# holstegelab/otter

Hardware: AMD Instinct MI355X
Metric: regions/sec (otter assemble) on synthetic TR BED+BAM, 1/2/4/8 MI355X (higher is better)
Workload: dtype i16

## Files before the change

### otter_amd/csrc/otg_chain.hpp

```cpp
#pragma once
#include "otg_common.hpp"
#include <cstddef>
#include <cstdlib>

struct OtgCounters {
  struct Tier { uint32_t ticket, overflow; };
  struct ExactEdit {
    uint32_t wf_ticket, tier_ticket[OTG_MYERS_TIERS];
    Tier wide, last;
    struct Routes { uint32_t len[OTG_MYERS_TIERS + 1], wf_len; } routes;
  } exact_edit;
  struct ExactAffine {
    uint32_t seg[OTG_REG_TIERS + 2];
    uint32_t reg_overflow, reg_ticket[OTG_REG_TIERS], bound_ticket;
    Tier a, b, c;
    unsigned long long visited, unused_, reg_timing[7];
  } exact_affine;
  struct AdaptiveEdit { Tier packed1024, packed4096, packed16384, bytes2048, bytes16384, last; } adaptive_edit;
  struct AdaptiveAffine { Tier win256, win1024, win4096, bytes1024, last; } adaptive_affine;
};
static_assert(offsetof(OtgCounters, exact_affine.visited) % 8 == 0 && offsetof(OtgCounters, exact_affine.reg_timing) % 8 == 0, "64-bit atomics need 8-byte alignment");
static_assert(offsetof(OtgCounters, exact_affine.reg_timing) - offsetof(OtgCounters, exact_affine.visited) == 16, "wfa_affine_reg.hip adds its clock sums at visited + 2 .. visited + 8");
static_assert(sizeof(OtgCounters::ExactEdit::Routes) <= 16 * sizeof(uint32_t), "ctx->edit_hist holds 16 words per kind of pass");

template <class G>
G* otg_counters(otg_ctx* ctx, G OtgCounters::*group, size_t bytes = sizeof(G))
{
  const bool fresh = !ctx->pool[SLOT_COUNTERS].p;
  OtgCounters* c = (OtgCounters*)otg_slot(ctx, SLOT_COUNTERS, sizeof(OtgCounters));
  if (!c) return nullptr;
  ctx->last_chain = (int)((const char*)&(c->*group) - (const char*)c);
  const hipError_t e = fresh ? hipMemsetAsync(c, 0, sizeof(OtgCounters), ctx->stream) : hipMemsetAsync(&(c->*group), 0, bytes, ctx->stream);
  if (e != hipSuccess) { otg_fail(ctx, OTG_ERR_HIP, "zeroing the chain counters failed"); return nullptr; }
  return &(c->*group);
}
inline unsigned long long* otg_affine_visited(otg_ctx* ctx) { OtgCounters* c = (OtgCounters*)ctx->pool[SLOT_COUNTERS].p; return c ? &c->exact_affine.visited : nullptr; }

inline int otg_timer_add(otg_ctx* ctx, float* kernel_ms, uint64_t* launches)
{
  if (!kernel_ms) return OTG_OK;
  HIP_TRY(ctx, hipEventSynchronize(ctx->ev1));
  float ms = 0;
  HIP_TRY(ctx, hipEventElapsedTime(&ms, ctx->ev0, ctx->ev1));
  *kernel_ms += ms;
  if (launches) *launches += 1;
  return OTG_OK;
}

struct OtgTodo {
  const uint32_t *list, *n; uint32_t imm;
  void next(const uint32_t* gave_up, const uint32_t* len) { list = gave_up; n = len; imm = 0; }
};

inline int otg_env_int(const char* name, int dflt) { const char* v = getenv(name); return v ? atoi(v) : dflt; }
inline bool otg_env_set(const char* name) { return getenv(name) != nullptr; }
// ... 1 lines not shown
```

### otter_amd/csrc/wfa_affine.hip

```cpp
#include "wfa_affine_common.hpp"
#include "wfa_affine_reg.hpp"
#include "otg_chain.hpp"
#include "otg_match_queue.hpp"
#include <algorithm>
#include <cstdlib>
#include <mutex>
#include <vector>

using namespace otg_affine;

namespace {

template <int WPB>
__global__ __launch_bounds__(WPB * 64) void wfa_affine_kernel(
    const uint8_t* __restrict__ arena, const otg_align_task* __restrict__ tasks,
    const uint32_t* __restrict__ todo, const uint32_t* __restrict__ n_todo_ptr, uint32_t n_todo_imm,
    int xs, int oes, int es, int g,
    int32_t* __restrict__ scores, const uint64_t* __restrict__ cig_off, uint32_t* __restrict__ cig_len,
    uint8_t* __restrict__ cig_arena, uint64_t* __restrict__ cells,
    uint32_t* __restrict__ ticket, uint32_t* __restrict__ n_overflow, uint32_t* __restrict__ overflow_list,
    AffWs ws)
{
  constexpr int QCAP = 2048;
  __shared__ int s_lo[WPB][3][64];
// ... 707 lines not shown
  const uint32_t a = seg[0], n = seg[1] - seg[0];
  for (uint32_t i = blockIdx.x * blockDim.x + threadIdx.x; i < n; i += gridDim.x * blockDim.x) out[i] = sorted[a + i];
  if (blockIdx.x == 0 && threadIdx.x == 0) *n_out = n;
}

}

int otg_launch_affine(otg_ctx* ctx, const uint8_t* d_arena, const otg_align_task* d_tasks, uint32_t n_tasks,
                      int x, int o, int e, int32_t* d_scores, const uint64_t* d_cig_off, uint32_t* d_cig_len,
                      uint8_t* d_cig_arena, uint64_t* d_cells)
{
  return otg_launch_affine_todo(ctx, d_arena, d_tasks, nullptr, nullptr, n_tasks, x, o, e, d_scores, d_cig_off, d_cig_len, d_cig_arena, d_cells);
}

int otg_launch_affine_todo(otg_ctx* ctx, const uint8_t* d_arena, const otg_align_task* d_tasks, const uint32_t* d_todo,
                           const uint32_t* d_n_todo, uint32_t n_tasks, int x, int o, int e, int32_t* d_scores,
                           const uint64_t* d_cig_off, uint32_t* d_cig_len, uint8_t* d_cig_arena, uint64_t* d_cells,
                           float* kernel_ms, uint64_t* launches)
{
  if (n_tasks == 0) return OTG_OK;
  ctx->affine_last = {};
  if (ctx->heur_strategy == OTG_HEURISTIC_WFADAPTIVE)
    return otg_launch_affine_adaptive_todo(ctx, d_arena, d_tasks, d_todo, d_n_todo, n_tasks, x, o, e, d_scores, d_cig_off, d_cig_len, d_cig_arena, d_cells,
                                           kernel_ms, launches);
  int g, xs, oes, es;
  if (int rc = affine_penalties(ctx, x, o, e, &g, &xs, &oes, &es)) return rc;
  OtgCounters::ExactAffine* const cnt = otg_counters(ctx, &OtgCounters::exact_affine, offsetof(OtgCounters::ExactAffine, visited));
  uint32_t* todo = (uint32_t*)otg_slot(ctx, SLOT_TODO, 4 * (size_t)n_tasks * sizeof(uint32_t));
  if (!cnt || !todo) return OTG_ERR_HIP;

  const size_t maxlen = ((size_t)ctx->max_seq_len + 4095) & ~(size_t)4095;
  AffWs ws = aff_ws_common(maxlen, xs, oes, es);
  ws.dbg = otg_env_set("OTG_DEBUG") ? 1 : 0; ws.visited = &cnt->visited;
  aff_ws_layout(ws, true);

  static const bool no_v3 = otg_env_set("OTG_NO_AFFINE_V3");
  static const bool no_bound = otg_env_set("OTG_NO_AFFINE_BOUND");
  static const int reg_mask_env = otg_env_int("OTG_AFFINE_REG", 31);
  static const int shape_env = otg_env_int("OTG_REG_SHAPE", 0);
  const int shape[OTG_REG_TIERS] = {(shape_env / 10000) % 10, (shape_env / 1000) % 10, (shape_env / 100) % 10, (shape_env / 10) % 10, shape_env % 10};
  const bool bounded = !no_v3 && es == 1 && xs == 2 && oes == 4 && !no_bound;
  int reg_mask = !bounded ? 0 : (maxlen <= 4096 ? (reg_mask_env & ~16) : reg_mask_env) & 31;

  constexpr int NWA = 4;
  constexpr int WPB = 4;
  AffWs wsA = ws, wsB = ws, wsC = ws, wr[OTG_REG_TIERS];
  uint32_t wavesA = 0, wavesB = 0, gridC = 2, blocks[OTG_REG_TIERS] = {0, 0, 0, 0, 0};
  const uint32_t ncu = (uint32_t)ctx->n_cu;
  {
    std::lock_guard<std::mutex> alloc_lock(otg_device_mutex(ctx->device));
    size_t free_b = 0, total_b = 0;
    HIP_TRY(ctx, hipMemGetInfo(&free_b, &total_b));
    const size_t budget = std::min<size_t>((size_t)(total_b * 0.2), (size_t)((free_b + ctx->pool[SLOT_WF_WS].cap) * 0.8));
    auto fit = [&](uint32_t& nwaves, size_t& slab) {
      while (nwaves > 1 && (ws.off_slab + slab) * (size_t)nwaves > budget) {
        if (slab > ((size_t)4 << 20)) slab /= 2; else nwaves = (nwaves + 1) / 2;
      }
    };
    auto diamond_slab = [&](size_t window) { return std::min<size_t>((size_t)(0.2 * (double)maxlen * (double)maxlen), window * window * 5 / 8) + (1 << 16); };
    wavesA = ncu * 2; size_t slabA = diamond_slab(4096);
    fit(wavesA, slabA);
    aff_ws_slab(wsA, slabA);
    wavesB = maxlen > 8192 ? ncu : ncu / 2; size_t slabB = diamond_slab(12288);
    fit(wavesB, slabB);
    aff_ws_slab(wsB, slabB);
    size_t slabC = std::min<size_t>((size_t)2 * maxlen * (size_t)(ws.nrows), budget / (gridC * WPB));
// ... 162 lines not shown
      std::vector<uint32_t> ids;
      if (d_todo) {
        if (d_n_todo) HIP_TRY(ctx, hipMemcpy(&n_live, d_n_todo, 4, hipMemcpyDeviceToHost)); else n_live = n_tasks;
        ids.resize(n_live);
        if (n_live) HIP_TRY(ctx, hipMemcpy(ids.data(), d_todo, (size_t)n_live * 4, hipMemcpyDeviceToHost));
      } else { n_live = n_tasks; ids.resize(n_live); for (uint32_t i = 0; i < n_live; ++i) ids[i] = i; }
      double su2 = 0, ss2 = 0; uint64_t hist[6] = {0, 0, 0, 0, 0, 0}, n_ok = 0;
      for (uint32_t q = 0; q < n_live; ++q) {
        const int32_t U = hb[ids[q]], sc = hs[ids[q]];
        if (U < 0 || U >= 0x40000000 || sc <= 0) continue;
        const double u = (double)U * g, r = u / (double)sc;
        su2 += u * u; ss2 += (double)sc * sc; ++n_ok;
        ++hist[r <= 1.0 ? 0 : r <= 1.02 ? 1 : r <= 1.05 ? 2 : r <= 1.1 ? 3 : r <= 1.2 ? 4 : 5];
      }
      if (n_ok) fprintf(stderr, "[otg] affine: bound / final score over %llu alignments: == 1: %.1f %%, <= 1.02: %.1f %%, <= 1.05: %.1f %%, <= 1.1: %.1f %%, <= 1.2: %.1f %%, above: %.1f %%; diamond cells outside the exact score's diamond: %.1f %%\n",
                        (unsigned long long)n_ok, 100.0 * hist[0] / n_ok, 100.0 * hist[1] / n_ok, 100.0 * hist[2] / n_ok, 100.0 * hist[3] / n_ok, 100.0 * hist[4] / n_ok, 100.0 * hist[5] / n_ok,
                        100.0 * (su2 - ss2) / su2);
    }
    if (h.reg_overflow && dbg_bound && bounded && reg_mask) {
      const uint32_t nshow = std::min<uint32_t>(h.reg_overflow, 24u);
      std::vector<uint32_t> ids(nshow);
      HIP_TRY(ctx, hipMemcpy(ids.data(), todo + 3 * (size_t)n_tasks, nshow * sizeof(uint32_t), hipMemcpyDeviceToHost));
      for (uint32_t i = 0; i < nshow; ++i) {
        otg_align_task t; int32_t U = 0, sc = 0;
        HIP_TRY(ctx, hipMemcpy(&t, d_tasks + ids[i], sizeof(t), hipMemcpyDeviceToHost));
        HIP_TRY(ctx, hipMemcpy(&U, dbg_bound + ids[i], sizeof(U), hipMemcpyDeviceToHost));
        HIP_TRY(ctx, hipMemcpy(&sc, d_scores + ids[i], sizeof(sc), hipMemcpyDeviceToHost));
        fprintf(stderr, "[otg] affine:   left its register tier: task %u, pattern %u, text %u, ends-free %d (pattern begin / end %d / %d, text begin / end %d / %d), bound %d, score %d\n",
                ids[i], t.pattern_len, t.text_len, t.endsfree, t.pattern_begin_free, t.pattern_end_free, t.text_begin_free, t.text_end_free, U, sc);
      }
    }
#ifdef OTG_REG_TIMING
    const unsigned long long* tm = h.reg_timing;
    HIP_TRY(ctx, hipMemsetAsync(cnt->reg_timing, 0, sizeof(h.reg_timing), ctx->stream));
    if (tm[5]) fprintf(stderr, "[otg] register tiers, clock ticks per wave and score: preamble %.0f sweep %.0f (%.2f slot visits) drain+fold %.0f exports %.0f barrier %.0f; %llu wave-scores\n",
                       (double)tm[0] / tm[5], (double)tm[1] / tm[5], (double)tm[6] / tm[5], (double)tm[2] / tm[5], (double)tm[3] / tm[5], (double)tm[4] / tm[5], tm[5]);
#endif
  }
  return otg_timer_add(ctx, kernel_ms, launches);
}

extern "C" int otg_affine_last_routing(otg_ctx* ctx, uint32_t n_tasks, int32_t* bound_out, int8_t* routed_out, int8_t* finished_out,
                                       uint32_t* counts_out, uint32_t* lists_out)
{
  const char* const who = "otg_affine_last_routing";
  if (!ctx) return otg_fail(nullptr, OTG_ERR_ARG, "%s: NULL context", who);
  if (!bound_out || !routed_out || !finished_out || !counts_out != !lists_out) return otg_fail(ctx, OTG_ERR_ARG, "%s: NULL argument", who);
  const otg_ctx::AffineLast& L = ctx->affine_last;
  if (ctx->heur_strategy != OTG_HEURISTIC_NONE) return otg_fail(ctx, OTG_ERR_ARG, "%s: the context's heuristic is WFadaptive; only the exact gap-affine chain is accounted for", who);
  if (ctx->last_chain != (int)offsetof(OtgCounters, exact_affine) || !ctx->pool[SLOT_COUNTERS].p || !ctx->pool[SLOT_TODO].p)
    return otg_fail(ctx, OTG_ERR_ARG, "%s: the last tier chain launched on this context was not the exact gap-affine chain", who);
  if (n_tasks == 0 || n_tasks != L.n_tasks) return otg_fail(ctx, OTG_ERR_ARG, "%s: the last gap-affine launch had %u tasks, not %u", who, L.n_tasks, n_tasks);
  if (L.sublist) return otg_fail(ctx, OTG_ERR_ARG, "%s: the last gap-affine launch worked on a list of task slots (the region pipeline's), not on a whole batch", who);
  if (ctx->pool[SLOT_TODO].cap < 4 * (size_t)n_tasks * sizeof(uint32_t) || (L.bounded && ctx->pool[SLOT_BT_POOL].cap < (size_t)n_tasks * sizeof(int32_t)))
    return otg_fail(ctx, OTG_ERR_ARG, "%s: the workspaces of the last gap-affine launch have been released", who);
  if (!L.scores_at || L.scores_at != ctx->pool[SLOT_SCORES].p || ctx->pool[SLOT_SCORES].cap < (size_t)n_tasks * sizeof(int32_t))
    return otg_fail(ctx, OTG_ERR_ARG, "%s: the scores of the last gap-affine launch are not in the context's score buffer (any more)", who);
  HIP_TRY(ctx, hipSetDevice(ctx->device));
  HIP_TRY(ctx, hipStreamSynchronize(ctx->stream));
  OtgCounters::ExactAffine c;
  HIP_TRY(ctx, hipMemcpy(&c, &((const OtgCounters*)ctx->pool[SLOT_COUNTERS].p)->exact_affine, sizeof(c), hipMemcpyDeviceToHost));
  std::vector<uint32_t> lists(4 * (size_t)n_tasks);
  HIP_TRY(ctx, hipMemcpy(lists.data(), ctx->pool[SLOT_TODO].p, lists.size() * sizeof(uint32_t), hipMemcpyDeviceToHost));
  std::vector<int32_t> sc(n_tasks);
  HIP_TRY(ctx, hipMemcpy(sc.data(), ctx->pool[SLOT_SCORES].p, (size_t)n_tasks * sizeof(int32_t), hipMemcpyDeviceToHost));
  if (!L.hbm_tiers) c.a.overflow = c.b.overflow = 0;
  if (!L.reg_mask) { for (uint32_t& x : c.seg) x = 0; c.reg_overflow = 0; }
  const uint32_t rest = c.seg[OTG_REG_TIERS + 1] - c.seg[OTG_REG_TIERS];
  bool sane = c.a.overflow <= n_tasks && c.b.overflow <= n_tasks && c.reg_overflow <= n_tasks && c.seg[OTG_REG_TIERS + 1] <= n_tasks;
// ... 28 lines not shown
```

### otter_amd/csrc/wfa_affine_common.hpp

```cpp
#pragma once
#include "otg_common.hpp"
#include <type_traits>

namespace otg_affine {

struct AffWs {
  uint8_t* base;
  size_t stride;
  size_t off_rowtab, off_rev, off_slab;
  size_t slab_bytes;
  int capa;
  int rm, ri;
  int nrows;
  size_t rev_cap;
  int dbg;
  unsigned long long* visited;
};

using lds_i16 = __attribute__((address_space(3))) int16_t;
using lds_u16 = __attribute__((address_space(3))) uint16_t;
using lds_u32 = __attribute__((address_space(3))) uint32_t;
using lds_u8 = __attribute__((address_space(3))) uint8_t;

__device__ __forceinline__ int imax(int a, int b) { return a > b ? a : b; }
__device__ __forceinline__ int imin(int a, int b) { return a < b ? a : b; }

constexpr int BT_ROWS = 64, BT_COLS = 32;
template <bool SHIFTED, class Eq>
__device__ bool backtrace_unpack(const uint8_t* P, int pl, const uint8_t* T, int tl, int s_end, int k_end, int xs, int oes, int es,
                                 const int64_t* rowtab, const uint8_t* slab, uint8_t* rev, size_t rev_cap, uint8_t* out, int lane,
                                 int32_t* score_out, uint32_t* len_out, int g, volatile lds_u32* win, Eq eq)
{
  uint32_t nrev = 0;
  int k0;
  {
    int s = s_end, k = k_end, comp = 0;
    int ws0 = -1, wk0 = 0;
    volatile lds_u8* win8 = (volatile lds_u8*)win;
    constexpr int MARGIN = SHIFTED ? 1 : 0;
    while (s > 0 || comp != 0) {
      if (ws0 < 0 || ws0 - s >= BT_ROWS || s > ws0 || k - MARGIN < wk0 || k + MARGIN >= wk0 + BT_COLS) {
        ws0 = s; wk0 = k - BT_COLS / 2;
        const int r = ws0 - lane;
        uint32_t w[8] = {0, 0, 0, 0, 0, 0, 0, 0};
        if (r >= 0) {
          const int64_t rb = rowtab[r];
          if (rb != -1) __builtin_memcpy(w, slab + rb + wk0, 32);
        }
// ... 142 lines not shown
```

### otter_amd/csrc/wfa_affine_reg.hip

```cpp
#include "wfa_affine_common.hpp"
#include "wfa_affine_reg.hpp"
#include <cstdlib>

using namespace otg_affine;

namespace {

typedef short otg_short2 __attribute__((ext_vector_type(2)));
typedef unsigned short otg_ushort2 __attribute__((ext_vector_type(2)));

template <int I, int N, class F> __device__ __forceinline__ void static_for(F&& f)
{
  if constexpr (I < N) { f(std::integral_constant<int, I>{}); static_for<I + 1, N>(f); }
}
__device__ __forceinline__ otg_short2 as_s2(uint32_t a) { otg_short2 x; __builtin_memcpy(&x, &a, 4); return x; }
__device__ __forceinline__ otg_ushort2 as_u2(uint32_t a) { otg_ushort2 x; __builtin_memcpy(&x, &a, 4); return x; }
__device__ __forceinline__ uint32_t from_s2(otg_short2 x) { uint32_t o; __builtin_memcpy(&o, &x, 4); return o; }
__device__ __forceinline__ uint32_t from_u2(otg_ushort2 x) { uint32_t o; __builtin_memcpy(&o, &x, 4); return o; }
__device__ __forceinline__ uint32_t pk_max_i16(uint32_t a, uint32_t b) { return from_s2(__builtin_elementwise_max(as_s2(a), as_s2(b))); }
__device__ __forceinline__ uint32_t pk_add_u16(uint32_t a, uint32_t b) { return from_u2(as_u2(a) + as_u2(b)); }
__device__ __forceinline__ uint32_t pk_sub_u16(uint32_t a, uint32_t b) { return from_u2(as_u2(a) - as_u2(b)); }
__device__ __forceinline__ uint32_t pk_sub_sat_i16(uint32_t a, uint32_t b) { return from_s2(__builtin_elementwise_sub_sat(as_s2(a), as_s2(b))); }
__device__ __forceinline__ uint32_t pk_ne01_u16(uint32_t a, uint32_t b)
{
  uint32_t d, r;
  asm("v_pk_sub_u16 %0, %1, %2" : "=v"(d) : "v"(a), "v"(b));
  asm("v_pk_min_u16 %0, %1, 1 op_sel_hi:[1,0]" : "=v"(r) : "v"(d));
  return r;
}
__device__ __forceinline__ void opaque_v(int& x) { asm volatile("" : "+v"(x)); }
__device__ __forceinline__ unsigned long long mk_eq(int a, int b) { return __builtin_amdgcn_sicmp(a, b, 32); }
__device__ __forceinline__ unsigned long long mk_gt(int a, int b) { return __builtin_amdgcn_sicmp(a, b, 38); }
__device__ __forceinline__ unsigned long long mk_ule(uint32_t a, uint32_t b) { return __builtin_amdgcn_uicmp(a, b, 37); }
__device__ __forceinline__ int sel(unsigned long long m, int a, int b) { int r; asm("v_cndmask_b32_e64 %0, %1, %2, %3" : "=v"(r) : "v"(b), "v"(a), "s"(m)); return r; }
__device__ __forceinline__ int sel0(unsigned long long m, int a) { int r; asm("v_cndmask_b32_e64 %0, 0, %1, %2" : "=v"(r) : "v"(a), "s"(m)); return r; }
__device__ __forceinline__ bool lane_in(unsigned long long m, int lane) { return ((m >> lane) & 1ull) != 0ull; }
__device__ __forceinline__ void opaque_v(uint32_t& x) { asm volatile("" : "+v"(x)); }
__device__ __forceinline__ void vset(uint32_t& dst, uint32_t src) { asm("v_mov_b32 %0, %1" : "+v"(dst) : "v"(src)); }
__device__ __forceinline__ void vswap(uint32_t& a, uint32_t& b) { asm("v_swap_b32 %0, %1" : "+v"(a), "+v"(b)); }
__device__ __forceinline__ uint32_t umin3(uint32_t a, uint32_t b, uint32_t c) { const uint32_t m = a < b ? a : b; return m < c ? m : c; }
__device__ __forceinline__ uint32_t pack16(int lo, int hi) { return __builtin_amdgcn_perm((uint32_t)hi, (uint32_t)lo, 0x05040100u); }
__device__ __forceinline__ uint64_t uniform64(uint64_t x)
{
  return ((uint64_t)(uint32_t)__builtin_amdgcn_readfirstlane((int)(x >> 32)) << 32) | (uint64_t)(uint32_t)__builtin_amdgcn_readfirstlane((int)(uint32_t)x);
}

#ifndef OTG_SCHED_FENCE
#define OTG_SCHED_FENCE() __builtin_amdgcn_sched_barrier(0)
#endif

template <int NW, int S2, int SEQB, int WPEU, int QCAP = 512, int LB = 2>
__global__ __launch_bounds__(NW == 1 ? 256 : NW * 64, WPEU) void wfa_affine_reg_kernel(
    const uint8_t* __restrict__ arena, const otg_align_task* __restrict__ tasks,
    const uint32_t* __restrict__ todo, const uint32_t* __restrict__ seg, int g,
    int32_t* __restrict__ scores, const uint64_t* __restrict__ cig_off, uint32_t* __restrict__ cig_len,
    uint8_t* __restrict__ cig_arena, uint64_t* __restrict__ cells,
    uint32_t* __restrict__ ticket, uint32_t* __restrict__ n_overflow, uint32_t* __restrict__ overflow_list,
    AffWs ws, const int32_t* __restrict__ bound, unsigned long long* __restrict__ visited)
{
  constexpr int xs = 2, oes = 4, es = 1;
  constexpr int CAP = NW * S2 * 128;
  constexpr int ALN = NW == 1 ? 4 : 1;
  constexpr int WAVES = NW == 1 ? 4 : NW;
  constexpr int GS = NW * S2;
  constexpr int FAILV = -2147483647 - 1;
  constexpr int NOCAND = 0x7fffffff;
  constexpr uint32_t NN = 0x80008000u;
  constexpr uint32_t ONE2 = 0x00010001u;
  constexpr int NUL16 = -32768;
  __shared__ uint32_t s_seq[ALN][SEQB / 4];
  __shared__ uint32_t s_patch[ALN][CAP / 2];
// ... 17 lines not shown
  uint8_t* slab = my + ws.off_slab;
  const uint32_t seg0 = seg[0], n_todo = seg[1] - seg[0];

  for (;;) {
    uint32_t tk;
    if (NW > 1) {
      if (wv == 0) MISC[0] = (int)otg_wave_atomic_add(ticket, 1u);
      __syncthreads();
      tk = (uint32_t)MISC[0];
    } else tk = otg_wave_atomic_add(ticket, 1u);
    if (tk >= n_todo) break;
    const uint32_t ti = (uint32_t)__builtin_amdgcn_readfirstlane((int)todo[seg0 + tk]);
    otg_align_task t = tasks[ti];
    t.pattern_off = uniform64(t.pattern_off); t.text_off = uniform64(t.text_off);
    t.pattern_len = (uint32_t)__builtin_amdgcn_readfirstlane((int)t.pattern_len); t.text_len = (uint32_t)__builtin_amdgcn_readfirstlane((int)t.text_len);
    t.pattern_begin_free = __builtin_amdgcn_readfirstlane(t.pattern_begin_free); t.pattern_end_free = __builtin_amdgcn_readfirstlane(t.pattern_end_free);
    t.text_begin_free = __builtin_amdgcn_readfirstlane(t.text_begin_free); t.text_end_free = __builtin_amdgcn_readfirstlane(t.text_end_free);
    t.endsfree = __builtin_amdgcn_readfirstlane(t.endsfree);
    const uint8_t* P = arena + t.pattern_off;
    const uint8_t* T = arena + t.text_off;
    const int pl = (int)t.pattern_len, tl = (int)t.text_len;
    const bool ef = t.endsfree != 0;
    const int pef = t.pattern_end_free, tef = t.text_end_free;
    const int kend = tl - pl;
    const int U = __builtin_amdgcn_readfirstlane(bound[ti]);
    const int elo = kend - (ef ? tef : 0), ehi = kend + (ef ? pef : 0);
    int lo0 = 0, hi0 = 0, kbase = 0;
    bool fail = U < 0 || U >= 0x40000000 || pl >= 32766 || tl >= 32766;
    const int offT = (pl + 15) / 16 + 3;
    if ((offT + (tl + 15) / 16 + 3) * 4 > SEQB) fail = true;
    if (!fail) {
      int need = 0;
      if (!affine_window(t, U, &kbase, &need, &lo0, &hi0) || need >= CAP) fail = true;
    }
    if (!fail) {
      for (int q = (NW == 1 ? lane : (int)threadIdx.x); q < CAP / 2; q += (NW == 1 ? 64 : NW * 64)) PT[q] = NN;
      if (NW > 1) for (int q = (int)threadIdx.x; q < 2 * XROW; q += NW * 64) XT[q] = NN;
      bool bad = false;
      auto pack = [&](const uint8_t* S, int len, int woff) {
        for (int q = (NW == 1 ? lane : (int)threadIdx.x); q < (len + 15) / 16; q += (NW == 1 ? 64 : NW * 64)) {
          uint32_t w = 0;
#pragma unroll
          for (int j = 0; j < 2; ++j) {
            const int b0 = 16 * q + 8 * j;
            const uint64_t x = b0 < len + 8 ? otg_load8(S + (b0 < len ? b0 : len)) : 0ull;
#pragma unroll
            for (int t2 = 0; t2 < 8; ++t2) {
              const uint32_t c = (uint32_t)(x >> (8 * t2)) & 0xffu;
              const uint32_t code = (c >> 1) & 3u;
              if (b0 + t2 < len && c != ((0x47544341u >> (8 * code)) & 0xffu)) bad = true;
              w |= code << (2 * (8 * j + t2));
            }
          }
          SQ[woff + q] = w;
        }
      };
      pack(P, pl, 0);
      pack(T, tl, offT);
      if ((NW == 1 ? lane : (int)threadIdx.x) < 3) { const int q3 = NW == 1 ? lane : (int)threadIdx.x; SQ[(pl + 15) / 16 + q3] = 0; SQ[offT + (tl + 15) / 16 + q3] = 0; }
      if (NW > 1) { if (threadIdx.x == 0) MISC[2] = 0; __syncthreads(); if (bad) MISC[2] = 1; __syncthreads(); fail = MISC[2] != 0; }
      else fail = __ballot(bad) != 0ull;
    }
    if (NW > 1) __syncthreads();
    __builtin_amdgcn_fence(__ATOMIC_SEQ_CST, "workgroup");
    auto ld32b = [&](int woff, int pos) -> uint64_t {
      const int w = woff + (pos >> 4);
// ... 27 lines not shown
#pragma nounroll
      for (int i = 0; i < nb; ++i) {
        if (m >= rem) break;
        const uint64_t x = ld32b(0, v + m) ^ ld32b(offT, h + m);
        if (x) { m += (int)(__builtin_ctzll(x) >> 1); break; }
        m += 32;
      }
      return m < rem ? m : rem;
    };
    auto wave_match = [&](int v, int h, int rem) -> int {
      int total = 0;
      while (total < rem) {
        const int off = total + lane * 32;
        uint64_t x = ~0ull;
        if (off < rem) x = ld32b(0, v + off) ^ ld32b(offT, h + off);
        const int m = x ? (int)(__builtin_ctzll(x) >> 1) : 32;
        const unsigned long long stop = __ballot(m < 32);
        if (stop) { const int f = (int)__builtin_ctzll(stop); total += f * 32 + __builtin_amdgcn_readlane(m, f); break; }
        total += 2048;
      }
      return total < rem ? total : rem;
    };

    uint32_t M4[2][S2], M2[2][S2];
    uint32_t WI[S2], WD[S2];
    static_for<0, S2>([&](auto ic) __attribute__((always_inline)) { constexpr int i = decltype(ic)::value;
      M4[0][i] = NN; M2[0][i] = NN; M4[1][i] = NN; M2[1][i] = NN; WI[i] = NN; WD[i] = NN;
      opaque_v(M4[0][i]); opaque_v(M2[0][i]); opaque_v(M4[1][i]); opaque_v(M2[1][i]); });
    uint32_t slab_top = 0;
    const uint32_t slab_cap = ws.slab_bytes > 0xfff00000ull ? 0xfff00000u : (uint32_t)ws.slab_bytes;
    int s_end = -1, k_end = 0;
    int r1lo = 1, r1hi = 0, r2lo = 1, r2hi = 0, r3lo = 1, r3hi = 0, r4lo = 1, r4hi = 0, idlo = 1, idhi = 0;
    uint32_t xlv = NN, xrv = NN;
    const int xe = kend - kbase;

    int lane2 = 2 * lane, kb = __builtin_amdgcn_readfirstlane(kbase);
    const int nul16v = NUL16;
#ifdef OTG_REG_TIMING
    unsigned long long tm_pre = 0, tm_sweep = 0, tm_drain = 0, tm_exp = 0, tm_bar = 0, tm_n = 0, tm_vis = 0, tm_last = __builtin_amdgcn_s_memtime();
#define OTG_TM(acc) { const unsigned long long now_ = __builtin_amdgcn_s_memtime(); acc += now_ - tm_last; tm_last = now_; }
#else
#define OTG_TM(acc)
#endif
    for (int s = 0; !fail; ++s) {
      if (s >= ws.nrows) { fail = true; break; }
      asm volatile("" : "+v"(lane2));
      asm volatile("" : "+s"(kb));
      int xes = xe;
      asm volatile("" : "+s"(xes));
      int lo, hi;
      if (s == 0) { lo = lo0; hi = hi0; }
      else {
        lo = 1 << 30; hi = -(1 << 30);
        if (r2hi >= r2lo) { lo = imin(lo, r2lo); hi = imax(hi, r2hi); }
        if (r4hi >= r4lo) { lo = imin(lo, r4lo - 1); hi = imax(hi, r4hi + 1); }
        if (idhi >= idlo) { lo = imin(lo, idlo - 1); hi = imax(hi, idhi + 1); }
        if (lo < -pl) lo = -pl;
        if (hi > tl) hi = tl;
        if (hi >= lo) {
          const int room = U - s;
          lo = imax(lo, elo - room); hi = imin(hi, ehi + room);
          if (room < 0 || hi < lo) { fail = true; break; }
        }
      }
      lo = __builtin_amdgcn_readfirstlane(lo); hi = __builtin_amdgcn_readfirstlane(hi);
      r4lo = r3lo; r4hi = r3hi; r3lo = r2lo; r3hi = r2hi; r2lo = r1lo; r2hi = r1hi;
      int cand = NOCAND;
      int j0 = 1, j1 = 0;
      if (hi < lo) {
        r1lo = 1; r1hi = 0; idlo = 1; idhi = 0;
        rowtab[s] = -1;
        if (s > 2 * (oes + es * (pl + tl)) + 8) { fail = true; break; }
      } else {
      r1lo = lo; r1hi = hi;
      const int xlo = lo - kbase, xhi = hi - kbase;
      if (xlo < 2 || xhi + 3 >= CAP) { fail = true; break; }
      j0 = (xlo - 1) >> 7; j1 = (xhi + 1) >> 7;
      const int width = (j1 - j0 + 1) * 128;
      if (slab_top + (uint32_t)width > slab_cap) { fail = true; break; }
      uint8_t* brow = slab + slab_top - 128 * j0;
      rowtab[s] = (int64_t)slab_top - (int64_t)(kbase + 128 * j0);
      slab_top += (uint32_t)width;
      int qn = 0;
      auto drain = [&]() {
        int pass = 0;
        while (qn > 0) {
          if (qn <= 4 && pass > 0) {
            for (int e = 0; e < qn; ++e) {
              const uint32_t ent = (uint32_t)__builtin_amdgcn_readfirstlane((int)QU[e]);
              const int x = (int)(ent & 0xffffu), h = (int)(ent >> 16), kk = kbase + x, v = h - kk;
              const int m = wave_match(v, h, imin(pl - v, tl - h));
              const int hf = h + m, vf = v + m;
              PT16[x] = (uint16_t)hf;
              if (ef ? ((hf >= tl && pl - vf <= pef) || (vf >= pl && tl - hf <= tef)) : (x == xe && hf >= tl)) cand = imin(cand, kk);
            }
            qn = 0;
            break;
          }
          int wq = 0;
          for (int q0 = 0; q0 < qn; q0 += 64) {
            const bool act = q0 + lane < qn;
            int x = 0, kk = 0, h = 0, v = 0;
            bool more = false, fin = false;
            if (act) {
              const uint32_t ent = QU[q0 + lane];
              x = (int)(ent & 0xffffu); h = (int)(ent >> 16); kk = kbase + x; v = h - kk;
              const int rem = imin(pl - v, tl - h);
              int m, full;
              if (pass == 0) { m = match_n(v, h, rem, 2); full = 64; }
              else { m = match_n(v, h, rem, 8); full = 256; }
              v += m; h += m;
              more = (m == full) && v < pl && h < tl;
              if (!more) {
                PT16[x] = (uint16_t)h;
                fin = ef ? ((h >= tl && pl - v <= pef) || (v >= pl && tl - h <= tef)) : (x == xe && h >= tl);
              }
            }
            const unsigned long long fm = __ballot(fin);
            if (fm) {
              int kc = fin ? kk : NOCAND;
              kc = -otg_wave_max_i32(-kc);
              cand = imin(cand, kc);
            }
            const unsigned long long mm = __ballot(more);
            if (more) {
              const int rank = (int)__builtin_amdgcn_mbcnt_hi((uint32_t)(mm >> 32), __builtin_amdgcn_mbcnt_lo((uint32_t)mm, 0u));
              QU[wq + rank] = (uint32_t)x | ((uint32_t)h << 16);
            }
            wq += __builtin_popcountll(mm);
          }
          qn = wq; ++pass;
        }
      };
      constexpr int QFULL = 2 * QCAP;
      auto push2 = [&](bool moreE, bool moreO, unsigned long long mE, unsigned long long mO, int xE, int hE, int hO) {
        if (mE | mO) {
          if (qn + 128 > QCAP) { qn = QFULL; return; }
          const int nE = __builtin_popcountll(mE);
          if (moreE) {
// ... 88 lines not shown
          if ((mmE | mmO) != 0ull) {
            const unsigned long long selO = mmO & ~mmE;
            const int h2 = sel(selO, hO, hE);
            const int v2 = h2 - sel(selO, kE + 1, kE);
            const int rv2 = pl - v2, rh2 = tl - h2;
            int m2nd;
            if constexpr (LB > 0) { const Ld3 p2 = ld3(0, v2), t2 = ld3(offT, h2); OTG_SCHED_FENCE(); m2nd = imin(probe_of(p2, v2, t2, h2), imin(rv2, rh2)); }
            else m2nd = imin(probe32(v2, h2), imin(rv2, rh2));
            const unsigned long long m2m = mk_eq(m2nd, 32) & mk_gt(rv2, 32) & mk_gt(rh2, 32);
            hO += sel0(selO, m2nd); hE += sel0(mmE, m2nd);
            mmO &= mmE | m2m; mmE &= m2m;
          }
          M4[0][i] = m2;
          M2[0][i] = pack16(sel(vmE, hE, nul16v), sel(vmO, hO, nul16v));
          if (ef) {
            const int hp = pl + kE;
            if ((mk_eq(hE, tl) | mk_eq(hE, hp) | mk_eq(hO, tl) | mk_eq(hO, hp + 1)) != 0ull) {
              const bool fE = lane_in(vmE & ~mmE, lane) && fin_ef(hE, hE - kE), fO = lane_in(vmO & ~mmO, lane) && fin_ef(hO, hO - kE - 1);
              const unsigned long long fm = __ballot(fE || fO);
              if (fm) { int kc = fE ? kE : (fO ? kE + 1 : NOCAND); kc = -otg_wave_max_i32(-kc); cand = imin(cand, kc); }
            }
          } else if ((xes >> 7) == gi) {
            const bool odd = (xes & 1) != 0;
            const int hx = __builtin_amdgcn_readlane(sel(odd ? (vmO & ~mmO) : (vmE & ~mmE), odd ? hO : hE, -1), (xes & 127) >> 1);
            if (hx >= tl) cand = kend;
          }
          if ((mmE | mmO) != 0ull) push2(lane_in(mmE, lane), lane_in(mmO, lane), mmE, mmO, xE, hE, hO);
        });
      }
      if (s == 0) static_for<0, S2>([&](auto ic) __attribute__((always_inline)) { constexpr int i = decltype(ic)::value; M4[0][i] = NN; opaque_v(M4[0][i]); });
      OTG_TM(tm_sweep);
#ifdef OTG_REG_TIMING
      tm_n += 1; tm_vis += (unsigned long long)(NW == 1 ? (j1 - j0 + 1) : ((j1 - ww + NW) / NW - (j0 - ww + NW - 1) / NW));
#endif
      if (qn >= QFULL) cand = FAILV;
      else if (qn > 0) {
        drain();
        static_for<0, S2>([&](auto ic) __attribute__((always_inline)) { constexpr int i = decltype(ic)::value;
          const int gi = NW == 1 ? i : i * NW + ww;
          if (gi < j0 || gi > j1) return;
          const int pi = 64 * gi + (lane2 >> 1);
          const uint32_t pw = PT[pi];
          if (__ballot(pw != NN)) {
            M2[0][i] = pk_max_i16(M2[0][i], pw);
            PT[pi] = NN;
          }
        });
      }
      idlo = s == 0 ? 1 : lo; idhi = s == 0 ? 0 : hi;
      OTG_TM(tm_drain);
      }
      cand = __builtin_amdgcn_readfirstlane(cand);
      if (NW > 1) {
        const int np = ((s + 1) & 1) * XROW;
        if (lane == 0 || lane == 63) {
          volatile lds_u32* dst = XT + np + (lane == 63 ? 0 : GS + 2) + ww + 1;
          static_for<0, S2>([&](auto ic) __attribute__((always_inline)) { constexpr int i = decltype(ic)::value;
            dst[i * NW] = pk_max_i16(M4[1][i], lane == 63 ? WI[i] : WD[i]); });
          if (lane == 0) XT[np + 2 * (GS + 2) + ww] = (uint32_t)cand;
        }
        OTG_TM(tm_exp);
        __syncthreads();
        xlv = XT[np + lane];
        xrv = XT[np + GS + 4 + lane];
        const int cv = (int)XT[np + 2 * (GS + 2) + (lane & (WAVES - 1))];
        int gc = NOCAND;
#pragma unroll
        for (int w2 = 0; w2 < NW; ++w2) { const int c2 = __builtin_amdgcn_readlane(cv, w2); gc = c2 < gc ? c2 : gc; }
        cand = __builtin_amdgcn_readfirstlane(gc);
        OTG_TM(tm_bar);
      }
      if (cand == FAILV) fail = true;
      else if (cand != NOCAND) { s_end = s; k_end = cand; }
      static_for<0, S2>([&](auto ic) __attribute__((always_inline)) { constexpr int i = decltype(ic)::value;
        vswap(M4[0][i], M4[1][i]);
        vswap(M2[0][i], M2[1][i]); });
      if (s_end >= 0) break;
    }

#ifdef OTG_REG_TIMING
    if (visited && lane == 0) {
      atomicAdd(visited + 2, tm_pre); atomicAdd(visited + 3, tm_sweep); atomicAdd(visited + 4, tm_drain); atomicAdd(visited + 5, tm_exp);
      atomicAdd(visited + 6, tm_bar); atomicAdd(visited + 7, tm_n); atomicAdd(visited + 8, tm_vis);
    }
#endif
    if (NW > 1 && wv != 0) continue;
    if (fail || s_end < 0) {
      const uint32_t q = otg_wave_atomic_add(n_overflow, 1u);
      overflow_list[q] = ti;
      continue;
    }
    __builtin_amdgcn_fence(__ATOMIC_SEQ_CST, "agent");
    if (!backtrace_unpack<true>(P, pl, T, tl, s_end, k_end, xs, oes, es, rowtab, slab, rev, ws.rev_cap, cig_arena + cig_off[ti], lane, &scores[ti], &cig_len[ti], g,
                                (volatile lds_u32*)&s_queue[wv][0], EqPacked{(volatile lds_u32*)&s_seq[al][0], offT})) continue;
    if (cells) cells[ti] = affine_cells(t, xs, oes, s_end);
    if (visited && lane == 0) atomicAdd(visited, (unsigned long long)slab_top);
  }
}

}

void otg_affine_reg_geometry(int tier, int shape, int* aln_per_block, int* blocks_per_cu)
{
  int a = 4, b = 4;
  switch (tier * 10 + shape) {
    case 0: a = 4; b = 4; break;
    case 1: a = 1; b = 10; break;
    case 10: a = 4; b = 3; break;
    case 11: a = 4; b = 4; break;
    case 12: a = 1; b = 8; break;
    case 20: a = 1; b = 8; break;
    case 21: a = 4; b = 3; break;
    case 22: a = 4; b = 2; break;
    case 30: a = 1; b = 4; break;
    case 31: a = 1; b = 3; break;
    case 40: a = 1; b = 2; break;
// ... 36 lines not shown
```

Before: 18060.

## Re-anchor register-tier affine diagonal window to keep band inside capacity

```diff
diff --git a/otter_amd/csrc/otg_chain.hpp b/otter_amd/csrc/otg_chain.hpp
--- a/otter_amd/csrc/otg_chain.hpp
+++ b/otter_amd/csrc/otg_chain.hpp
@@ -14,13 +14,13 @@
     uint32_t seg[OTG_REG_TIERS + 2];
     uint32_t reg_overflow, reg_ticket[OTG_REG_TIERS], bound_ticket;
     Tier a, b, c;
-    unsigned long long visited, unused_, reg_timing[7];
+    unsigned long long visited, reg_live, reg_timing[7];
   } exact_affine;
   struct AdaptiveEdit { Tier packed1024, packed4096, packed16384, bytes2048, bytes16384, last; } adaptive_edit;
   struct AdaptiveAffine { Tier win256, win1024, win4096, bytes1024, last; } adaptive_affine;
 };
 static_assert(offsetof(OtgCounters, exact_affine.visited) % 8 == 0 && offsetof(OtgCounters, exact_affine.reg_timing) % 8 == 0, "64-bit atomics need 8-byte alignment");
-static_assert(offsetof(OtgCounters, exact_affine.reg_timing) - offsetof(OtgCounters, exact_affine.visited) == 16, "wfa_affine_reg.hip adds its clock sums at visited + 2 .. visited + 8");
+static_assert(offsetof(OtgCounters, exact_affine.reg_timing) - offsetof(OtgCounters, exact_affine.visited) == 16, "wfa_affine_reg.hip adds its live-diagonal sum at visited + 1, its clock sums at visited + 2 .. visited + 8");
 static_assert(sizeof(OtgCounters::ExactEdit::Routes) <= 16 * sizeof(uint32_t), "ctx->edit_hist holds 16 words per kind of pass");
 
 template <class G>
diff --git a/otter_amd/csrc/otg_reanchor.hpp b/otter_amd/csrc/otg_reanchor.hpp
--- /dev/null
+++ b/otter_amd/csrc/otg_reanchor.hpp
@@ -0,0 +1,33 @@
+#pragma once
+
+#if defined(__HIPCC__) || defined(__CUDACC__)
+#define OTG_REANCHOR_FN __host__ __device__ inline
+#else
+#define OTG_REANCHOR_FN inline
+#endif
+
+constexpr int OTG_REANCHOR_LAG = 8;
+constexpr int OTG_REANCHOR_FLOOR = 4;
+constexpr int OTG_REANCHOR_MAX_SHIFT = 63;
+
+OTG_REANCHOR_FN bool otg_reanchor_fits(int xlo, int xhi, int cap) { return xlo >= 2 && xhi + 3 < cap; }
+
+OTG_REANCHOR_FN int otg_reanchor_shift(int xlo, int xhi, int cap)
+{
+  constexpr int TOP = OTG_REANCHOR_FLOOR + 2 * OTG_REANCHOR_LAG - 1;
+  if ((unsigned)(xlo - OTG_REANCHOR_FLOOR) < (unsigned)(2 * OTG_REANCHOR_LAG) && xhi + 3 < cap) return 0;
+  const int maxlo = cap - 4 - (xhi - xlo);
+  if (maxlo < 2) return 0;
+  const int lower = maxlo > OTG_REANCHOR_FLOOR ? OTG_REANCHOR_FLOOR : 2, upper = maxlo < TOP ? maxlo : TOP;
+  int d = 0;
+  if (xlo < lower) d = -((upper - xlo) >> 1);
+  else if (xlo > upper) d = (xlo - lower) >> 1;
+  return d < -OTG_REANCHOR_MAX_SHIFT ? -OTG_REANCHOR_MAX_SHIFT : d > OTG_REANCHOR_MAX_SHIFT ? OTG_REANCHOR_MAX_SHIFT : d;
+}
+
+OTG_REANCHOR_FN int otg_reanchor_first(int width_m1, int cap)
+{
+  constexpr int TOP = OTG_REANCHOR_FLOOR + 2 * OTG_REANCHOR_LAG - 1;
+  const int maxlo = cap - 4 - width_m1;
+  return maxlo < TOP ? maxlo : TOP;
+}
diff --git a/otter_amd/csrc/wfa_affine.hip b/otter_amd/csrc/wfa_affine.hip
--- a/otter_amd/csrc/wfa_affine.hip
+++ b/otter_amd/csrc/wfa_affine.hip
@@ -763,6 +763,8 @@
   const size_t maxlen = ((size_t)ctx->max_seq_len + 4095) & ~(size_t)4095;
   AffWs ws = aff_ws_common(maxlen, xs, oes, es);
   ws.dbg = otg_env_set("OTG_DEBUG") ? 1 : 0; ws.visited = &cnt->visited;
+  static const bool reanchor_env = otg_env_int("OTG_AFFINE_REANCHOR", 1) != 0;
+  ws.reanchor = reanchor_env ? 1 : 0;
   aff_ws_layout(ws, true);
 
   static const bool no_v3 = otg_env_set("OTG_NO_AFFINE_V3");
@@ -991,9 +993,11 @@
     }
 #ifdef OTG_REG_TIMING
     const unsigned long long* tm = h.reg_timing;
-    HIP_TRY(ctx, hipMemsetAsync(cnt->reg_timing, 0, sizeof(h.reg_timing), ctx->stream));
-    if (tm[5]) fprintf(stderr, "[otg] register tiers, clock ticks per wave and score: preamble %.0f sweep %.0f (%.2f slot visits) drain+fold %.0f exports %.0f barrier %.0f; %llu wave-scores\n",
-                       (double)tm[0] / tm[5], (double)tm[1] / tm[5], (double)tm[6] / tm[5], (double)tm[2] / tm[5], (double)tm[3] / tm[5], (double)tm[4] / tm[5], tm[5]);
+    HIP_TRY(ctx, hipMemsetAsync(&cnt->reg_live, 0, sizeof(h.reg_live) + sizeof(h.reg_timing), ctx->stream));
+    if (tm[5]) fprintf(stderr, "[otg] register tiers, clock ticks per wave and score: preamble %.0f sweep %.0f (%.2f slot visits) drain+fold %.0f exports %.0f barrier %.0f; %llu wave-scores; "
+                       "live diagonals %llu in %llu slot visits of 128 (live / visited %.3f)\n",
+                       (double)tm[0] / tm[5], (double)tm[1] / tm[5], (double)tm[6] / tm[5], (double)tm[2] / tm[5], (double)tm[3] / tm[5], (double)tm[4] / tm[5], tm[5],
+                       h.reg_live, tm[6], tm[6] ? (double)h.reg_live / (128.0 * (double)tm[6]) : 0.0);
 #endif
   }
   return otg_timer_add(ctx, kernel_ms, launches);
diff --git a/otter_amd/csrc/wfa_affine_common.hpp b/otter_amd/csrc/wfa_affine_common.hpp
--- a/otter_amd/csrc/wfa_affine_common.hpp
+++ b/otter_amd/csrc/wfa_affine_common.hpp
@@ -14,6 +14,7 @@
   int nrows;
   size_t rev_cap;
   int dbg;
+  int reanchor;
   unsigned long long* visited;
 };
 
diff --git a/otter_amd/csrc/wfa_affine_reg.hip b/otter_amd/csrc/wfa_affine_reg.hip
--- a/otter_amd/csrc/wfa_affine_reg.hip
+++ b/otter_amd/csrc/wfa_affine_reg.hip
@@ -1,5 +1,6 @@
 #include "wfa_affine_common.hpp"
 #include "wfa_affine_reg.hpp"
+#include "otg_reanchor.hpp"
 #include <cstdlib>
 
 using namespace otg_affine;
@@ -37,6 +38,34 @@
 __device__ __forceinline__ bool lane_in(unsigned long long m, int lane) { return ((m >> lane) & 1ull) != 0ull; }
 __device__ __forceinline__ void opaque_v(uint32_t& x) { asm volatile("" : "+v"(x)); }
 __device__ __forceinline__ void vset(uint32_t& dst, uint32_t src) { asm("v_mov_b32 %0, %1" : "+v"(dst) : "v"(src)); }
+__device__ __forceinline__ void perm12(uint32_t& a0, uint32_t& a1, uint32_t& a2, uint32_t& a3, uint32_t& a4, uint32_t& a5,
+                                       uint32_t& b0, uint32_t& b1, uint32_t& b2, uint32_t& b3, uint32_t& b4, uint32_t& b5, int addr, int d)
+{
+  asm volatile("s_cmp_eq_u32 %13, 0\n\ts_cbranch_scc1 .Lotg_perm%=\n\t"
+               "ds_bpermute_b32 %0, %12, %0\n\tds_bpermute_b32 %1, %12, %1\n\tds_bpermute_b32 %2, %12, %2\n\tds_bpermute_b32 %3, %12, %3\n\t"
+               "ds_bpermute_b32 %4, %12, %4\n\tds_bpermute_b32 %5, %12, %5\n\tds_bpermute_b32 %6, %12, %6\n\tds_bpermute_b32 %7, %12, %7\n\t"
+               "ds_bpermute_b32 %8, %12, %8\n\tds_bpermute_b32 %9, %12, %9\n\tds_bpermute_b32 %10, %12, %10\n\tds_bpermute_b32 %11, %12, %11\n\t"
+               "s_waitcnt lgkmcnt(0)\n.Lotg_perm%=:"
+               : "+v"(a0), "+v"(a1), "+v"(a2), "+v"(a3), "+v"(a4), "+v"(a5), "+v"(b0), "+v"(b1), "+v"(b2), "+v"(b3), "+v"(b4), "+v"(b5)
+               : "v"(addr), "s"(d) : "scc");
+}
+template <bool DOWN>
+__device__ __forceinline__ void patch12(uint32_t& a0, uint32_t& a1, uint32_t& a2, uint32_t& a3, uint32_t& a4, uint32_t& a5,
+                                        uint32_t& b0, uint32_t& b1, uint32_t& b2, uint32_t& b3, uint32_t& b4, uint32_t& b5,
+                                        uint32_t n0, uint32_t n1, uint32_t n2, uint32_t n3, uint32_t n4, uint32_t n5, unsigned long long own, int d)
+{
+#define OTG_PATCH12_BODY                                                                                                                                  \
+               "v_cndmask_b32_e64 %0, %6, %0, %18\n\tv_cndmask_b32_e64 %1, %7, %1, %18\n\tv_cndmask_b32_e64 %2, %8, %2, %18\n\t"                         \
+               "v_cndmask_b32_e64 %3, %9, %3, %18\n\tv_cndmask_b32_e64 %4, %10, %4, %18\n\tv_cndmask_b32_e64 %5, %11, %5, %18\n\t"                       \
+               "v_cndmask_b32_e64 %6, %12, %6, %18\n\tv_cndmask_b32_e64 %7, %13, %7, %18\n\tv_cndmask_b32_e64 %8, %14, %8, %18\n\t"                      \
+               "v_cndmask_b32_e64 %9, %15, %9, %18\n\tv_cndmask_b32_e64 %10, %16, %10, %18\n\tv_cndmask_b32_e64 %11, %17, %11, %18\n"                    \
+               ".Lotg_patch%=:"                                                                                                                           \
+               : "+v"(a0), "+v"(a1), "+v"(a2), "+v"(a3), "+v"(a4), "+v"(a5), "+v"(b0), "+v"(b1), "+v"(b2), "+v"(b3), "+v"(b4), "+v"(b5)                   \
+               : "v"(n0), "v"(n1), "v"(n2), "v"(n3), "v"(n4), "v"(n5), "s"(own), "s"(d) : "scc"
+  if constexpr (DOWN) asm volatile("s_cmp_lt_i32 %19, 1\n\ts_cbranch_scc1 .Lotg_patch%=\n\t" OTG_PATCH12_BODY);
+  else asm volatile("s_cmp_gt_i32 %19, -1\n\ts_cbranch_scc1 .Lotg_patch%=\n\t" OTG_PATCH12_BODY);
+#undef OTG_PATCH12_BODY
+}
 __device__ __forceinline__ void vswap(uint32_t& a, uint32_t& b) { asm("v_swap_b32 %0, %1" : "+v"(a), "+v"(b)); }
 __device__ __forceinline__ uint32_t umin3(uint32_t a, uint32_t b, uint32_t c) { const uint32_t m = a < b ? a : b; return m < c ? m : c; }
 __device__ __forceinline__ uint32_t pack16(int lo, int hi) { return __builtin_amdgcn_perm((uint32_t)hi, (uint32_t)lo, 0x05040100u); }
@@ -120,6 +149,7 @@
     if (!fail) {
       int need = 0;
       if (!affine_window(t, U, &kbase, &need, &lo0, &hi0) || need >= CAP) fail = true;
+      if (NW == 1 && ws.reanchor) kbase = lo0 - otg_reanchor_first(hi0 - lo0, CAP);
     }
     if (!fail) {
       for (int q = (NW == 1 ? lane : (int)threadIdx.x); q < CAP / 2; q += (NW == 1 ? 64 : NW * 64)) PT[q] = NN;
@@ -213,12 +243,11 @@
     int s_end = -1, k_end = 0;
     int r1lo = 1, r1hi = 0, r2lo = 1, r2hi = 0, r3lo = 1, r3hi = 0, r4lo = 1, r4hi = 0, idlo = 1, idhi = 0;
     uint32_t xlv = NN, xrv = NN;
-    const int xe = kend - kbase;
 
     int lane2 = 2 * lane, kb = __builtin_amdgcn_readfirstlane(kbase);
     const int nul16v = NUL16;
 #ifdef OTG_REG_TIMING
-    unsigned long long tm_pre = 0, tm_sweep = 0, tm_drain = 0, tm_exp = 0, tm_bar = 0, tm_n = 0, tm_vis = 0, tm_last = __builtin_amdgcn_s_memtime();
+    unsigned long long tm_pre = 0, tm_sweep = 0, tm_drain = 0, tm_exp = 0, tm_bar = 0, tm_n = 0, tm_vis = 0, tm_live = 0, tm_last = __builtin_amdgcn_s_memtime();
 #define OTG_TM(acc) { const unsigned long long now_ = __builtin_amdgcn_s_memtime(); acc += now_ - tm_last; tm_last = now_; }
 #else
 #define OTG_TM(acc)
@@ -227,8 +256,6 @@
       if (s >= ws.nrows) { fail = true; break; }
       asm volatile("" : "+v"(lane2));
       asm volatile("" : "+s"(kb));
-      int xes = xe;
-      asm volatile("" : "+s"(xes));
       int lo, hi;
       if (s == 0) { lo = lo0; hi = hi0; }
       else {
@@ -246,6 +273,28 @@
       }
       lo = __builtin_amdgcn_readfirstlane(lo); hi = __builtin_amdgcn_readfirstlane(hi);
       r4lo = r3lo; r4hi = r3hi; r3lo = r2lo; r3hi = r2hi; r2lo = r1lo; r2hi = r1hi;
+      if constexpr (NW == 1) {
+        int d = 0;
+        if (ws.reanchor && hi >= lo) d = otg_reanchor_shift(lo - kb, hi - kb, CAP);
+        d = __builtin_amdgcn_readfirstlane(d);
+        const int addr = (2 * lane2 + 4 * d) & 252;
+        const unsigned long long ownD = (1ull << ((64 - d) & 63)) - 1ull, ownU = ~0ull << (-d & 63);
+        uint32_t nnv = NN;
+        opaque_v(nnv);
+        static_for<0, S2 / 2>([&](auto ic) __attribute__((always_inline)) { constexpr int i = 2 * decltype(ic)::value;
+          perm12(M4[0][i], M2[0][i], M4[1][i], M2[1][i], WI[i], WD[i], M4[0][i + 1], M2[0][i + 1], M4[1][i + 1], M2[1][i + 1], WI[i + 1], WD[i + 1], addr, d); });
+        static_for<0, S2 / 2>([&](auto ic) __attribute__((always_inline)) { constexpr int i = 2 * decltype(ic)::value;
+          if constexpr (i + 2 < S2) patch12<true>(M4[0][i], M2[0][i], M4[1][i], M2[1][i], WI[i], WD[i], M4[0][i + 1], M2[0][i + 1], M4[1][i + 1], M2[1][i + 1], WI[i + 1], WD[i + 1],
+                                                  M4[0][i + 2], M2[0][i + 2], M4[1][i + 2], M2[1][i + 2], WI[i + 2], WD[i + 2], ownD, d);
+          else patch12<true>(M4[0][i], M2[0][i], M4[1][i], M2[1][i], WI[i], WD[i], M4[0][i + 1], M2[0][i + 1], M4[1][i + 1], M2[1][i + 1], WI[i + 1], WD[i + 1],
+                             nnv, nnv, nnv, nnv, nnv, nnv, ownD, d); });
+        static_for<0, S2 / 2>([&](auto ic) __attribute__((always_inline)) { constexpr int i = S2 - 1 - 2 * decltype(ic)::value;
+          if constexpr (i >= 2) patch12<false>(M4[0][i], M2[0][i], M4[1][i], M2[1][i], WI[i], WD[i], M4[0][i - 1], M2[0][i - 1], M4[1][i - 1], M2[1][i - 1], WI[i - 1], WD[i - 1],
+                                               M4[0][i - 2], M2[0][i - 2], M4[1][i - 2], M2[1][i - 2], WI[i - 2], WD[i - 2], ownU, d);
+          else patch12<false>(M4[0][i], M2[0][i], M4[1][i], M2[1][i], WI[i], WD[i], M4[0][i - 1], M2[0][i - 1], M4[1][i - 1], M2[1][i - 1], WI[i - 1], WD[i - 1],
+                              nnv, nnv, nnv, nnv, nnv, nnv, ownU, d); });
+        kb += 2 * d;
+      }
       int cand = NOCAND;
       int j0 = 1, j1 = 0;
       if (hi < lo) {
@@ -254,13 +303,16 @@
         if (s > 2 * (oes + es * (pl + tl)) + 8) { fail = true; break; }
       } else {
       r1lo = lo; r1hi = hi;
-      const int xlo = lo - kbase, xhi = hi - kbase;
+      const int xlo = lo - kb, xhi = hi - kb;
       if (xlo < 2 || xhi + 3 >= CAP) { fail = true; break; }
+      const int xe = kend - kb;
+      int xes = xe;
+      asm volatile("" : "+s"(xes));
       j0 = (xlo - 1) >> 7; j1 = (xhi + 1) >> 7;
       const int width = (j1 - j0 + 1) * 128;
       if (slab_top + (uint32_t)width > slab_cap) { fail = true; break; }
       uint8_t* brow = slab + slab_top - 128 * j0;
-      rowtab[s] = (int64_t)slab_top - (int64_t)(kbase + 128 * j0);
+      rowtab[s] = (int64_t)slab_top - (int64_t)(kb + 128 * j0);
       slab_top += (uint32_t)width;
       int qn = 0;
       auto drain = [&]() {
@@ -269,7 +321,7 @@
           if (qn <= 4 && pass > 0) {
             for (int e = 0; e < qn; ++e) {
               const uint32_t ent = (uint32_t)__builtin_amdgcn_readfirstlane((int)QU[e]);
-              const int x = (int)(ent & 0xffffu), h = (int)(ent >> 16), kk = kbase + x, v = h - kk;
+              const int x = (int)(ent & 0xffffu), h = (int)(ent >> 16), kk = kb + x, v = h - kk;
               const int m = wave_match(v, h, imin(pl - v, tl - h));
               const int hf = h + m, vf = v + m;
               PT16[x] = (uint16_t)hf;
@@ -285,7 +337,7 @@
             bool more = false, fin = false;
             if (act) {
               const uint32_t ent = QU[q0 + lane];
-              x = (int)(ent & 0xffffu); h = (int)(ent >> 16); kk = kbase + x; v = h - kk;
+              x = (int)(ent & 0xffffu); h = (int)(ent >> 16); kk = kb + x; v = h - kk;
               const int rem = imin(pl - v, tl - h);
               int m, full;
               if (pass == 0) { m = match_n(v, h, rem, 2); full = 64; }
@@ -440,6 +492,7 @@
       OTG_TM(tm_sweep);
 #ifdef OTG_REG_TIMING
       tm_n += 1; tm_vis += (unsigned long long)(NW == 1 ? (j1 - j0 + 1) : ((j1 - ww + NW) / NW - (j0 - ww + NW - 1) / NW));
+      if (NW == 1 || ww == 0) tm_live += (unsigned long long)(hi - lo + 3);
 #endif
       if (qn >= QFULL) cand = FAILV;
       else if (qn > 0) {
@@ -489,7 +542,7 @@
 #ifdef OTG_REG_TIMING
     if (visited && lane == 0) {
       atomicAdd(visited + 2, tm_pre); atomicAdd(visited + 3, tm_sweep); atomicAdd(visited + 4, tm_drain); atomicAdd(visited + 5, tm_exp);
-      atomicAdd(visited + 6, tm_bar); atomicAdd(visited + 7, tm_n); atomicAdd(visited + 8, tm_vis);
+      atomicAdd(visited + 6, tm_bar); atomicAdd(visited + 7, tm_n); atomicAdd(visited + 8, tm_vis); atomicAdd(visited + 1, tm_live);
     }
 #endif
     if (NW > 1 && wv != 0) continue;
```

Result: no change. 17920 (-0.8%).
